# gongweibao/FleetX

Measured on AMD Instinct MI355X. Metric: tokens/sec (whole node) GPT-3 6.7B hybrid-parallel at 1/2/4/8 MI355X, higher is better.
Workload: dtype bf16; 1 GPU; model=gpt3-6.7B, global_batch=8, seq_len=1024, parallelism=dp1, micro_batch=8, hip_graph=True, grad_reduce_dtype=float32, recompute=False

## Files before the change

csrc/kernels/norm_eltwise.hip:

```cpp
#include "fx_api.h"
#include "fx_common.h"

namespace {

struct DropCfg {
  uint32_t klo, khi, thr;
  float scale;
  int enabled;
  const uint64_t* salt;
};

__device__ __forceinline__ DropCfg resolve_drop(DropCfg d) {
  if (d.enabled && d.salt != nullptr) {
    const uint64_t k = salt_key(((uint64_t)d.khi << 32) | d.klo, *d.salt);
    d.klo = (uint32_t)k;
    d.khi = (uint32_t)(k >> 32);
  }
  return d;
}

__device__ __forceinline__ float drop_apply(float v, uint64_t idx, const DropCfg& d) {
  if (!d.enabled) return v;
  uint32_t h = elem_rand_pair(idx, d.klo, d.khi);
  uint32_t r = (idx & 1) ? (h >> 16) : (h & 0xffffu);
  return r >= d.thr ? v * d.scale : 0.f;
}

__device__ __forceinline__ void drop_apply8(float* v, uint64_t idx0, const DropCfg& d) {
  if (!d.enabled) return;
#pragma unroll
  for (int q = 0; q < 4; ++q) {
    const uint32_t h = elem_rand_pair(idx0 + 2 * q, d.klo, d.khi);
    v[2 * q] = (h & 0xffffu) >= d.thr ? v[2 * q] * d.scale : 0.f;
    v[2 * q + 1] = (h >> 16) >= d.thr ? v[2 * q + 1] * d.scale : 0.f;
  }
}

template <typename T, int VPT, bool MASK = false>
__global__ __launch_bounds__(256) void add_ln_fwd_kernel(
    const uint16_t* __restrict__ x, const uint16_t* __restrict__ bias,
    const uint16_t* __restrict__ residual, const uint16_t* __restrict__ gamma,
    const uint16_t* __restrict__ beta, uint16_t* __restrict__ s_out,
    uint16_t* __restrict__ y, float* __restrict__ mean_out, float* __restrict__ rstd_out,
    int rows, int h, float eps, DropCfg drop_) {
  const DropCfg drop = resolve_drop(drop_);
  const int lane = threadIdx.x & 63;
  const int row = blockIdx.x * 4 + (threadIdx.x >> 6);
  if (row >= rows) return;
  const size_t base = (size_t)row * h;
  uint4 xr[VPT], rr[VPT], br[VPT];
#pragma unroll
  for (int i = 0; i < VPT; ++i) {
    const int c = (i * 64 + lane) * 8;
    xr[i] = rr[i] = br[i] = make_uint4(0, 0, 0, 0);
    if (!MASK || c < h) xr[i] = *reinterpret_cast<const uint4*>(x + base + c);
  }
  if (residual) {
#pragma unroll
    for (int i = 0; i < VPT; ++i) {
      const int c = (i * 64 + lane) * 8;
      if (!MASK || c < h) rr[i] = *reinterpret_cast<const uint4*>(residual + base + c);
    }
  }
  if (bias) {
#pragma unroll
    for (int i = 0; i < VPT; ++i) {
      const int c = (i * 64 + lane) * 8;
      if (!MASK || c < h) br[i] = *reinterpret_cast<const uint4*>(bias + c);
    }
  }
  float v[VPT][8];
  float sum = 0.f;
#pragma unroll
  for (int i = 0; i < VPT; ++i) {
    const int c = (i * 64 + lane) * 8;
    if (MASK && c >= h) {
#pragma unroll
      for (int j = 0; j < 8; ++j) v[i][j] = 0.f;
      continue;
    }
    unpack8<T>(xr[i], v[i]);
    if (bias) {
      float b[8];
      unpack8<T>(br[i], b);
#pragma unroll
      for (int j = 0; j < 8; ++j) v[i][j] += b[j];
    }
    if (drop.enabled) {
      drop_apply8(v[i], base + c, drop);
    }
    if (residual) {
      float r[8];
      unpack8<T>(rr[i], r);
#pragma unroll
      for (int j = 0; j < 8; ++j) v[i][j] += r[j];
    }
    if (s_out) {
      store8<T>(s_out + base + c, v[i]);
#pragma unroll
      for (int j = 0; j < 8; ++j) v[i][j] = round_to<T>(v[i][j]);
    }
#pragma unroll
    for (int j = 0; j < 8; ++j) sum += v[i][j];
  }
  const float mean = wave_sum(sum) / h;
  float var = 0.f;
#pragma unroll
  for (int i = 0; i < VPT; ++i) {
    if (MASK && (i * 64 + lane) * 8 >= h) continue;
#pragma unroll
    for (int j = 0; j < 8; ++j) {
      float d = v[i][j] - mean;
      var += d * d;
    }
  }
  const float rstd = rsqrtf(wave_sum(var) / h + eps);
#pragma unroll
  for (int i = 0; i < VPT; ++i) {
    const int c = (i * 64 + lane) * 8;
    if (MASK && c >= h) continue;
    float g[8], b[8], o[8];
    load8<T>(gamma + c, g);
    load8<T>(beta + c, b);
#pragma unroll
    for (int j = 0; j < 8; ++j) o[j] = (v[i][j] - mean) * rstd * g[j] + b[j];
    store8<T>(y + base + c, o);
  }
  if (lane == 0) {
    mean_out[row] = mean;
    rstd_out[row] = rstd;
  }
}

template <typename T>
__global__ __launch_bounds__(256) void add_ln_fwd_generic(
    const uint16_t* __restrict__ x, const uint16_t* __restrict__ bias,
    const uint16_t* __restrict__ residual, const uint16_t* __restrict__ gamma,
    const uint16_t* __restrict__ beta, uint16_t* __restrict__ s_out,
    uint16_t* __restrict__ y, float* __restrict__ mean_out, float* __restrict__ rstd_out,
    int rows, int h, float eps, DropCfg drop_) {
  const DropCfg drop = resolve_drop(drop_);
  const int lane = threadIdx.x & 63;
  const int row = blockIdx.x * 4 + (threadIdx.x >> 6);
  if (row >= rows) return;
  const size_t base = (size_t)row * h;
  const int nv = h / 8;
  auto value = [&](int c, float* v) {
    load8<T>(x + base + c, v);
    if (bias) {
      float b[8];
      load8<T>(bias + c, b);
      for (int j = 0; j < 8; ++j) v[j] += b[j];
    }
    if (drop.enabled)
      drop_apply8(v, base + c, drop);
    if (residual) {
      float r[8];
      load8<T>(residual + base + c, r);
      for (int j = 0; j < 8; ++j) v[j] += r[j];
    }
  };
  float sum = 0.f;
  for (int vi = lane; vi < nv; vi += 64) {
    float v[8];
    value(vi * 8, v);
    if (s_out) {
      store8<T>(s_out + base + vi * 8, v);
      for (int j = 0; j < 8; ++j) v[j] = round_to<T>(v[j]);
    }
    for (int j = 0; j < 8; ++j) sum += v[j];
  }
  const float mean = wave_sum(sum) / h;
  float var = 0.f;
  for (int vi = lane; vi < nv; vi += 64) {
    float v[8];
    if (s_out) load8<T>(s_out + base + vi * 8, v); else value(vi * 8, v);
    for (int j = 0; j < 8; ++j) { float d = v[j] - mean; var += d * d; }
  }
  const float rstd = rsqrtf(wave_sum(var) / h + eps);
  for (int vi = lane; vi < nv; vi += 64) {
    float v[8], g[8], b[8], o[8];
    if (s_out) load8<T>(s_out + base + vi * 8, v); else value(vi * 8, v);
    load8<T>(gamma + vi * 8, g);
    load8<T>(beta + vi * 8, b);
    for (int j = 0; j < 8; ++j) o[j] = (v[j] - mean) * rstd * g[j] + b[j];
    store8<T>(y + base + vi * 8, o);
  }
  if (lane == 0) { mean_out[row] = mean; rstd_out[row] = rstd; }
}

template <typename T, int VPT, bool MASK = false>
__global__ __launch_bounds__(256) void ln_bwd_row_kernel(
    const uint16_t* __restrict__ dy, const uint16_t* __restrict__ s,
    const float* __restrict__ mean_in, const float* __restrict__ rstd_in,
    const uint16_t* __restrict__ gamma, const uint16_t* __restrict__ ds_in,
    uint16_t* __restrict__ ds_out, uint16_t* __restrict__ dx_out, int rows, int h,
    DropCfg drop_) {
  const DropCfg drop = resolve_drop(drop_);
  const int lane = threadIdx.x & 63;
  const int row = blockIdx.x * 4 + (threadIdx.x >> 6);
  if (row >= rows) return;
  const size_t base = (size_t)row * h;
  const float mean = mean_in[row], rstd = rstd_in[row];
  float xh[VPT][8], gdy[VPT][8];
  float s1 = 0.f, s2 = 0.f;
#pragma unroll
  for (int i = 0; i < VPT; ++i) {
    const int c = (i * 64 + lane) * 8;
    if (MASK && c >= h) {
#pragma unroll
      for (int j = 0; j < 8; ++j) xh[i][j] = gdy[i][j] = 0.f;
      continue;
    }
    float a[8], g[8], d[8];
    load8<T>(s + base + c, a);
    load8<T>(gamma + c, g);
    load8<T>(dy + base + c, d);
#pragma unroll
    for (int j = 0; j < 8; ++j) {
      xh[i][j] = (a[j] - mean) * rstd;
      gdy[i][j] = d[j] * g[j];
      s1 += gdy[i][j];
      s2 += gdy[i][j] * xh[i][j];
    }
  }
  uint4 dr[VPT];
  if (ds_in) {
#pragma unroll
    for (int i = 0; i < VPT; ++i) {
      const int c = (i * 64 + lane) * 8;
      dr[i] = make_uint4(0, 0, 0, 0);
      if (!MASK || c < h) dr[i] = *reinterpret_cast<const uint4*>(ds_in + base + c);
    }
  }
  const float m1 = wave_sum(s1) / h, m2 = wave_sum(s2) / h;
#pragma unroll
  for (int i = 0; i < VPT; ++i) {
    const int c = (i * 64 + lane) * 8;
    if (MASK && c >= h) continue;
    float o[8];
#pragma unroll
    for (int j = 0; j < 8; ++j) o[j] = rstd * (gdy[i][j] - m1 - xh[i][j] * m2);
    if (ds_in) {
      float r[8];
      unpack8<T>(dr[i], r);
#pragma unroll
      for (int j = 0; j < 8; ++j) o[j] += r[j];
    }
    store8<T>(ds_out + base + c, o);
    if (drop.enabled) {
      drop_apply8(o, base + c, drop);
      store8<T>(dx_out + base + c, o);
    } else if (dx_out != ds_out) {
      store8<T>(dx_out + base + c, o);
    }
  }
}

template <typename T>
__global__ __launch_bounds__(256) void ln_bwd_row_generic(
    const uint16_t* __restrict__ dy, const uint16_t* __restrict__ s,
    const float* __restrict__ mean_in, const float* __restrict__ rstd_in,
    const uint16_t* __restrict__ gamma, const uint16_t* __restrict__ ds_in,
    uint16_t* __restrict__ ds_out, uint16_t* __restrict__ dx_out, int rows, int h,
    DropCfg drop_) {
  const DropCfg drop = resolve_drop(drop_);
  const int lane = threadIdx.x & 63;
  const int row = blockIdx.x * 4 + (threadIdx.x >> 6);
  if (row >= rows) return;
  const size_t base = (size_t)row * h;
  const float mean = mean_in[row], rstd = rstd_in[row];
  const int nv = h / 8;
  float s1 = 0.f, s2 = 0.f;
  for (int vi = lane; vi < nv; vi += 64) {
    float a[8], g[8], d[8];
    load8<T>(s + base + vi * 8, a);
    load8<T>(gamma + vi * 8, g);
    load8<T>(dy + base + vi * 8, d);
    for (int j = 0; j < 8; ++j) {
      float xh = (a[j] - mean) * rstd, gd = d[j] * g[j];
      s1 += gd;
      s2 += gd * xh;
    }
  }
  const float m1 = wave_sum(s1) / h, m2 = wave_sum(s2) / h;
  for (int vi = lane; vi < nv; vi += 64) {
    const int c = vi * 8;
    float a[8], g[8], d[8], o[8];
    load8<T>(s + base + c, a);
    load8<T>(gamma + c, g);
    load8<T>(dy + base + c, d);
    for (int j = 0; j < 8; ++j) o[j] = rstd * (d[j] * g[j] - m1 - (a[j] - mean) * rstd * m2);
    if (ds_in) {
      float r[8];
      load8<T>(ds_in + base + c, r);
      for (int j = 0; j < 8; ++j) o[j] += r[j];
    }
    store8<T>(ds_out + base + c, o);
    if (drop.enabled) {
      drop_apply8(o, base + c, drop);
      store8<T>(dx_out + base + c, o);
    } else if (dx_out != ds_out) {
      store8<T>(dx_out + base + c, o);
    }
  }
}

template <typename T, int VPT, int WPR, bool MASK, bool DB>
__global__ __launch_bounds__(256, 2) void ln_bwd_cols_kernel(
    const uint16_t* __restrict__ dy, const uint16_t* __restrict__ s,
    const float* __restrict__ mean_in, const float* __restrict__ rstd_in,
    const uint16_t* __restrict__ gamma, const uint16_t* __restrict__ ds_in,
    uint16_t* __restrict__ ds_out, uint16_t* __restrict__ dx_out, int rows, int h,
    int rows_per_group, float* __restrict__ part, DropCfg drop_) {
  constexpr int NG = 4 / WPR;
  __shared__ float red[4 * 512 * VPT];
  __shared__ float xs[2][4][2];
  const DropCfg drop = resolve_drop(drop_);
  const int lane = threadIdx.x & 63, w = threadIdx.x >> 6;
  const int grp = w / WPR, half = w % WPR;
  const int hw = h / WPR, cbase = half * hw;
  const int r0 = min(rows, (blockIdx.x * NG + grp) * rows_per_group);
  const int r1 = min(rows, r0 + rows_per_group);
  uint4 gp[VPT];
  float ag[VPT][8], ab[VPT][8], ax[DB ? VPT : 1][8];
#pragma unroll
  for (int i = 0; i < VPT; ++i) {
    const int c = (i * 64 + lane) * 8;
    gp[i] = (!MASK || c < hw) ? *reinterpret_cast<const uint4*>(gamma + cbase + c)
                              : make_uint4(0, 0, 0, 0);
#pragma unroll
    for (int j = 0; j < 8; ++j) {
      ag[i][j] = ab[i][j] = 0.f;
      if (DB) ax[i][j] = 0.f;
    }
  }
  for (int k = 0; k < rows_per_group; ++k) {
    const int r = r0 + k;
    const bool live = r < r1;
    if (WPR == 1 && !live) break;
    const size_t base = (size_t)(live ? r : 0) * h + cbase;
    uint4 ca[VPT], cd[VPT], cr[VPT];
    float mean = 0.f, rstd = 0.f, s1 = 0.f, s2 = 0.f;
    if (live) {
#pragma unroll
      for (int i = 0; i < VPT; ++i) {
        const int c = (i * 64 + lane) * 8;
        if (MASK && c >= hw) continue;
        ca[i] = *reinterpret_cast<const uint4*>(s + base + c);
        cd[i] = *reinterpret_cast<const uint4*>(dy + base + c);
      }
      if (ds_in) {
#pragma unroll
        for (int i = 0; i < VPT; ++i) {
          const int c = (i * 64 + lane) * 8;
          if (MASK && c >= hw) continue;
          cr[i] = *reinterpret_cast<const uint4*>(ds_in + base + c);
        }
      }
      mean = mean_in[r];
      rstd = rstd_in[r];
#pragma unroll
      for (int i = 0; i < VPT; ++i) {
        const int c = (i * 64 + lane) * 8;
        if (MASK && c >= hw) continue;
        float a[8], d[8], g[8];
        unpack8<T>(ca[i], a);
        unpack8<T>(cd[i], d);
        unpack8<T>(gp[i], g);
#pragma unroll
        for (int j = 0; j < 8; ++j) {
          const float xh = (a[j] - mean) * rstd, gd = d[j] * g[j];
          s1 += gd;
          s2 += gd * xh;
          ag[i][j] += d[j] * xh;
          ab[i][j] += d[j];
        }
      }
    }
    s1 = wave_sum(s1);
    s2 = wave_sum(s2);
    if constexpr (WPR > 1) {
      if (lane == 0) {
        xs[k & 1][w][0] = s1;
        xs[k & 1][w][1] = s2;
      }
      __syncthreads();
      s1 = xs[k & 1][WPR * grp][0];
      s2 = xs[k & 1][WPR * grp][1];
#pragma unroll
      for (int q = 1; q < WPR; ++q) {
        s1 += xs[k & 1][WPR * grp + q][0];
        s2 += xs[k & 1][WPR * grp + q][1];
      }
    }
    if (!live) continue;
    const float m1 = s1 / h, m2 = s2 / h;
#pragma unroll
    for (int i = 0; i < VPT; ++i) {
      const int c = (i * 64 + lane) * 8;
      if (MASK && c >= hw) continue;
      float a[8], d[8], g[8], o[8];
      unpack8<T>(ca[i], a);
      unpack8<T>(cd[i], d);
      unpack8<T>(gp[i], g);
#pragma unroll
      for (int j = 0; j < 8; ++j) o[j] = rstd * (d[j] * g[j] - m1 - (a[j] - mean) * rstd * m2);
      if (ds_in) {
        float rr[8];
        unpack8<T>(cr[i], rr);
#pragma unroll
        for (int j = 0; j < 8; ++j) o[j] += rr[j];
      }
      store8<T>(ds_out + base + c, o);
      if (drop.enabled) {
        drop_apply8(o, base + c, drop);
        store8<T>(dx_out + base + c, o);
      } else if (dx_out != ds_out) {
        store8<T>(dx_out + base + c, o);
      }
      if (DB) {
#pragma unroll
        for (int j = 0; j < 8; ++j) ax[i][j] += round_to<T>(o[j]);
      }
    }
  }
#pragma unroll
  for (int arr = 0; arr < (DB ? 3 : 2); ++arr) {
    __syncthreads();
#pragma unroll
    for (int i = 0; i < VPT; ++i) {
      const int c = (i * 64 + lane) * 8;
      if (MASK && c >= hw) continue;
#pragma unroll
      for (int j = 0; j < 8; ++j)
        red[grp * h + cbase + c + j] = arr == 0 ? ag[i][j] : arr == 1 ? ab[i][j] : ax[DB ? i : 0][j];
    }
    __syncthreads();
    float* out = part + ((size_t)arr * gridDim.x + blockIdx.x) * h;
    for (int c = threadIdx.x; c < h; c += 256) {
      float v = red[c];
#pragma unroll
      for (int q = 1; q < NG; ++q) v += red[q * h + c];
      out[c] = v;
    }
  }
}

struct LnColsOut {
  float* f32[3];
  uint16_t* t16[3];
  int acc[3];
};
template <typename T>
__global__ __launch_bounds__(256) void ln_cols_finalize_kernel(const float* __restrict__ part,
                                                               int G, int h, LnColsOut f) {
  __shared__ float tr[8][132];
  const int arr = blockIdx.y;
  const float* p = part + (size_t)arr * G * h;
  const int q = threadIdx.x & 31, sr = threadIdx.x >> 5;
  const int c0 = blockIdx.x * 128 + q * 4;
  floatx4 acc = {0.f, 0.f, 0.f, 0.f};
  if (c0 < h) {
    for (int k0 = sr; k0 < G; k0 += 128) {
      floatx4 v[16];
#pragma unroll
      for (int u = 0; u < 16; ++u) {
        const int k = k0 + 8 * u;
        v[u] = k < G ? *reinterpret_cast<const floatx4*>(p + (size_t)k * h + c0)
                     : floatx4{0.f, 0.f, 0.f, 0.f};
      }
#pragma unroll
      for (int u = 0; u < 16; ++u) acc += v[u];
    }
  }
#pragma unroll
  for (int j = 0; j < 4; ++j) tr[sr][q * 4 + j] = acc[j];
  __syncthreads();
  const int c = threadIdx.x, gc = blockIdx.x * 128 + c;
  if (c >= 128 || gc >= h) return;
  float sum = 0.f;
#pragma unroll
  for (int t = 0; t < 8; ++t) sum += tr[t][c];
  if (f.f32[arr]) f.f32[arr][gc] = f.acc[arr] ? f.f32[arr][gc] + sum : sum;
  if (f.t16[arr]) f.t16[arr][gc] = Elt<T>::from_f(sum);
}

typedef __attribute__((address_space(1))) float gf32;
typedef __attribute__((address_space(1))) int gi32;

__device__ __forceinline__ void st_part(float* p, float v) {
  __hip_atomic_store((gf32*)p, v, __ATOMIC_RELAXED, __HIP_MEMORY_SCOPE_AGENT);
}

struct ColFin {
  int* cnt;
  float* f32[2];
  uint16_t* t16[2];
  int acc[2];
};

template <typename T>
__device__ __forceinline__ void colsum_tail(const float* __restrict__ p0,
                                            const float* __restrict__ p1, int cols, int np,
                                            const ColFin& f) {
  __shared__ int last;
  asm volatile("s_waitcnt vmcnt(0)" ::: "memory");
  __syncthreads();
  if (threadIdx.x == 0) {
    const int t = __hip_atomic_fetch_add((gi32*)(f.cnt + 32 * blockIdx.x), 1, __ATOMIC_RELAXED,
                                         __HIP_MEMORY_SCOPE_AGENT);
    last = t == (int)gridDim.y - 1;
    if (last)
      __hip_atomic_store((gi32*)(f.cnt + 32 * blockIdx.x), 0, __ATOMIC_RELAXED,
                         __HIP_MEMORY_SCOPE_AGENT);
  }
  __syncthreads();
  if (!last) return;
  __builtin_amdgcn_fence(__ATOMIC_ACQUIRE, "wavefront");
  __shared__ float tr[8][132];
  const int q = threadIdx.x & 31, sr = threadIdx.x >> 5;
  const int c0 = blockIdx.x * 128 + q * 4;
  const int splits = gridDim.y;
  for (int which = 0; which < np; ++which) {
    const float* p = which ? p1 : p0;
    floatx4 s = {0.f, 0.f, 0.f, 0.f};
    if (c0 < cols) {
      const auto rs = __builtin_amdgcn_make_buffer_rsrc(const_cast<float*>(p), 0,
                                                        splits * cols * 4, 0x00020000);
      for (int k0 = sr; k0 < splits; k0 += 128) {
        floatx4 v[16];
#pragma unroll
        for (int u = 0; u < 16; ++u) {
          const int k = k0 + 8 * u;
          const uint32_t off = k < splits ? (uint32_t)(k * cols + c0) * 4u : 0x80000000u;
          v[u] = __builtin_bit_cast(floatx4, __builtin_amdgcn_raw_buffer_load_b128(rs, off, 0, 16));
        }
#pragma unroll
        for (int u = 0; u < 16; ++u) s += v[u];
      }
    }
#pragma unroll
    for (int j = 0; j < 4; ++j) tr[sr][q * 4 + j] = s[j];
    __syncthreads();
    const int c = threadIdx.x, gc = blockIdx.x * 128 + c;
    if (c < 128 && gc < cols) {
      float sum = 0.f;
#pragma unroll
      for (int t = 0; t < 8; ++t) sum += tr[t][c];
      if (f.f32[which]) f.f32[which][gc] = f.acc[which] ? f.f32[which][gc] + sum : sum;
      if (f.t16[which]) f.t16[which][gc] = Elt<T>::from_f(sum);
    }
    __syncthreads();
  }
}

template <typename T, int MODE>
__global__ __launch_bounds__(256) void coltile_partial_kernel(
    const uint16_t* __restrict__ a, const uint16_t* __restrict__ b,
    const float* __restrict__ mean, const float* __restrict__ rstd,
    float* __restrict__ p0, float* __restrict__ p1, int rows, int cols, int rows_per_split,
    ColFin fin) {
  __shared__ float red[2][16][129];
  const int tx = threadIdx.x & 15, ty = threadIdx.x >> 4;
  const int col = blockIdx.x * 128 + tx * 8;
  const int r0 = blockIdx.y * rows_per_split;
  const int r1 = min(rows, r0 + rows_per_split);
  float acc0[8], acc1[8];
#pragma unroll
  for (int j = 0; j < 8; ++j) acc0[j] = acc1[j] = 0.f;
  if (col < cols) {
    int r = r0 + ty;
    for (; r + 48 < r1; r += 64) {
      float va[4][8], vb[MODE == 0 ? 4 : 1][8], m[4], rs[4];
#pragma unroll
      for (int q = 0; q < 4; ++q) {
        const size_t off = (size_t)(r + 16 * q) * cols + col;
        load8<T>(a + off, va[q]);
        if (MODE == 0) {
          load8<T>(b + off, vb[q]);
          m[q] = mean[r + 16 * q];
          rs[q] = rstd[r + 16 * q];
        }
      }
#pragma unroll
      for (int q = 0; q < 4; ++q) {
#pragma unroll
        for (int j = 0; j < 8; ++j) {
          if (MODE == 0) {
            acc0[j] += va[q][j] * (vb[MODE == 0 ? q : 0][j] - m[q]) * rs[q];
            acc1[j] += va[q][j];
          } else {
            acc0[j] += va[q][j];
          }
        }
      }
    }
    for (; r < r1; r += 16) {
      const size_t off = (size_t)r * cols + col;
      float va[8];
      load8<T>(a + off, va);
      if (MODE == 0) {
        float vb[8];
        load8<T>(b + off, vb);
        const float m = mean[r], rs = rstd[r];
#pragma unroll
        for (int j = 0; j < 8; ++j) {
          acc0[j] += va[j] * (vb[j] - m) * rs;
          acc1[j] += va[j];
        }
      } else {
#pragma unroll
        for (int j = 0; j < 8; ++j) acc0[j] += va[j];
      }
    }
  }
#pragma unroll
  for (int j = 0; j < 8; ++j) {
    red[0][ty][tx * 8 + j] = acc0[j];
    red[1][ty][tx * 8 + j] = acc1[j];
  }
  __syncthreads();
  const int which = threadIdx.x >> 7, c = threadIdx.x & 127;
  if (MODE == 0 || which == 0) {
    float s = 0.f;
#pragma unroll
    for (int t = 0; t < 16; ++t) s += red[which][t][c];
    const int gc = blockIdx.x * 128 + c;
    if (gc < cols) st_part((which == 0 ? p0 : p1) + (size_t)blockIdx.y * cols + gc, s);
  }
  if (fin.cnt) colsum_tail<T>(p0, p1, cols, MODE == 0 ? 2 : 1, fin);
}

template <typename T>
__global__ void coltile_finalize_kernel(const float* __restrict__ p, int splits, int cols,
                                        float* __restrict__ out_f32, uint16_t* __restrict__ out_t,
                                        int accumulate) {
  const int c = blockIdx.x * blockDim.x + threadIdx.x;
  if (c >= cols) return;
  float a[8];
#pragma unroll
  for (int j = 0; j < 8; ++j) a[j] = 0.f;
  int k = 0;
  for (; k + 8 <= splits; k += 8) {
#pragma unroll
    for (int j = 0; j < 8; ++j) a[j] += p[(size_t)(k + j) * cols + c];
  }
  for (int j = 0; k + j < splits; ++j) a[j] += p[(size_t)(k + j) * cols + c];
  const float s = ((a[0] + a[1]) + (a[2] + a[3])) + ((a[4] + a[5]) + (a[6] + a[7]));
  if (out_f32) out_f32[c] = accumulate ? out_f32[c] + s : s;
  if (out_t) out_t[c] = Elt<T>::from_f(s);
}

template <typename T, bool ERF>
__global__ __launch_bounds__(256) void bias_gelu_fwd_kernel(
    const uint16_t* __restrict__ x, const uint16_t* __restrict__ bias, uint16_t* __restrict__ y,
    long n8, int cols) {
  for (long v = blockIdx.x * (long)blockDim.x + threadIdx.x; v < n8; v += (long)gridDim.x * blockDim.x) {
    const long off = v * 8;
    const int c = (int)(off % cols);
    float a[8], b[8];
    load8<T>(x + off, a);
    if (bias) load8<T>(bias + c, b);
#pragma unroll
    for (int j = 0; j < 8; ++j) {
      float t = a[j] + (bias ? b[j] : 0.f);
      a[j] = ERF ? gelu_erf(t) : gelu_tanh(t);
    }
    store8<T>(y + off, a);
  }
}

template <typename T, bool ERF>
__global__ __launch_bounds__(256) void bias_gelu_bwd_kernel(
    const uint16_t* __restrict__ dy, const uint16_t* __restrict__ x,
    const uint16_t* __restrict__ bias, uint16_t* __restrict__ dx, float* __restrict__ part,
    int rows, int cols, int rows_per_split, ColFin fin) {
  __shared__ float red[16][129];
  const int tx = threadIdx.x & 15, ty = threadIdx.x >> 4;
  const int col = blockIdx.x * 128 + tx * 8;
  const int r0 = blockIdx.y * rows_per_split;
  const int r1 = min(rows, r0 + rows_per_split);
  float acc[8];
#pragma unroll
  for (int j = 0; j < 8; ++j) acc[j] = 0.f;
  if (col < cols) {
    float b[8];
    if (bias) load8<T>(bias + col, b);
    else {
#pragma unroll
      for (int j = 0; j < 8; ++j) b[j] = 0.f;
    }
    for (int r = r0 + ty; r < r1; r += 16) {
      const size_t off = (size_t)r * cols + col;
      float g[8], a[8];
      load8<T>(dy + off, g);
      load8<T>(x + off, a);
#pragma unroll
      for (int j = 0; j < 8; ++j) {
        float t = a[j] + b[j];
        g[j] *= ERF ? gelu_erf_grad(t) : gelu_tanh_grad(t);
      }
      store8<T>(dx + off, g);
#pragma unroll
      for (int j = 0; j < 8; ++j) acc[j] += round_to<T>(g[j]);
    }
  }
#pragma unroll
  for (int j = 0; j < 8; ++j) red[ty][tx * 8 + j] = acc[j];
  __syncthreads();
  if (threadIdx.x < 128) {
    float s = 0.f;
#pragma unroll
    for (int t = 0; t < 16; ++t) s += red[t][threadIdx.x];
    const int gc = blockIdx.x * 128 + threadIdx.x;
    if (part && gc < cols) st_part(part + (size_t)blockIdx.y * cols + gc, s);
  }
  if (fin.cnt) colsum_tail<T>(part, nullptr, cols, 1, fin);
}

template <typename T>
__global__ __launch_bounds__(256) void bias_dropout_add_fwd_kernel(
    const uint16_t* __restrict__ x, const uint16_t* __restrict__ bias,
    const uint16_t* __restrict__ residual, uint16_t* __restrict__ out, long n8, int cols,
    DropCfg drop_) {
  const DropCfg drop = resolve_drop(drop_);
  for (long v = blockIdx.x * (long)blockDim.x + threadIdx.x; v < n8; v += (long)gridDim.x * blockDim.x) {
    const long off = v * 8;
    const int c = (int)(off % cols);
    float a[8];
    load8<T>(x + off, a);
    if (bias) {
      float b[8];
      load8<T>(bias + c, b);
#pragma unroll
      for (int j = 0; j < 8; ++j) a[j] += b[j];
    }
    drop_apply8(a, (uint64_t)off, drop);
    if (residual) {
      float r[8];
      load8<T>(residual + off, r);
#pragma unroll
      for (int j = 0; j < 8; ++j) a[j] += r[j];
    }
    store8<T>(out + off, a);
  }
}

template <typename T>
__global__ __launch_bounds__(256) void dropout_bwd_colsum_kernel(
    const uint16_t* __restrict__ dout, uint16_t* __restrict__ dx, float* __restrict__ part,
    int rows, int cols, int rows_per_split, DropCfg drop_, ColFin fin) {
  const DropCfg drop = resolve_drop(drop_);
  __shared__ float red[16][129];
  const int tx = threadIdx.x & 15, ty = threadIdx.x >> 4;
  const int col = blockIdx.x * 128 + tx * 8;
  const int r0 = blockIdx.y * rows_per_split;
  const int r1 = min(rows, r0 + rows_per_split);
  float acc[8];
#pragma unroll
  for (int j = 0; j < 8; ++j) acc[j] = 0.f;
  if (col < cols) {
    int r = r0 + ty;
    for (; r + 48 < r1; r += 64) {
      float g[4][8];
#pragma unroll
      for (int q = 0; q < 4; ++q) load8<T>(dout + (size_t)(r + 16 * q) * cols + col, g[q]);
#pragma unroll
      for (int q = 0; q < 4; ++q) {
        const size_t off = (size_t)(r + 16 * q) * cols + col;
        drop_apply8(g[q], off, drop);
        if (dx) {
          store8<T>(dx + off, g[q]);
#pragma unroll
          for (int j = 0; j < 8; ++j) g[q][j] = round_to<T>(g[q][j]);
        }
#pragma unroll
        for (int j = 0; j < 8; ++j) acc[j] += g[q][j];
      }
    }
    for (; r < r1; r += 16) {
      const size_t off = (size_t)r * cols + col;
      float g[8];
      load8<T>(dout + off, g);
      drop_apply8(g, off, drop);
      if (dx) {
        store8<T>(dx + off, g);
#pragma unroll
        for (int j = 0; j < 8; ++j) g[j] = round_to<T>(g[j]);
      }
#pragma unroll
      for (int j = 0; j < 8; ++j) acc[j] += g[j];
    }
  }
#pragma unroll
  for (int j = 0; j < 8; ++j) red[ty][tx * 8 + j] = acc[j];
  __syncthreads();
  if (threadIdx.x < 128) {
    float s = 0.f;
#pragma unroll
    for (int t = 0; t < 16; ++t) s += red[t][threadIdx.x];
    const int gc = blockIdx.x * 128 + threadIdx.x;
    if (part && gc < cols) st_part(part + (size_t)blockIdx.y * cols + gc, s);
  }
  if (fin.cnt) colsum_tail<T>(part, nullptr, cols, 1, fin);
}

template <typename T>
__global__ __launch_bounds__(256) void dropout_fwd_kernel(const uint16_t* __restrict__ x,
                                                          uint16_t* __restrict__ y, long n,
                                                          DropCfg drop_) {
  const DropCfg drop = resolve_drop(drop_);
  const long n8 = n / 8;
  for (long v = blockIdx.x * (long)blockDim.x + threadIdx.x; v < n8; v += (long)gridDim.x * blockDim.x) {
    const long off = v * 8;
    float a[8];
    load8<T>(x + off, a);
    drop_apply8(a, (uint64_t)off, drop);
    store8<T>(y + off, a);
  }
  for (long i = n8 * 8 + blockIdx.x * (long)blockDim.x + threadIdx.x; i < n;
       i += (long)gridDim.x * blockDim.x)
    y[i] = Elt<T>::from_f(drop_apply(Elt<T>::to_f(x[i]), (uint64_t)i, drop));
}

DropCfg make_drop(float p, uint64_t key, const void* salt) {
  DropCfg d;
  d.enabled = p > 0.f ? 1 : 0;
  d.klo = (uint32_t)(key & 0xffffffffu);
  d.khi = (uint32_t)(key >> 32);
  d.thr = (uint32_t)(p * 65536.0f + 0.5f);
  d.scale = p < 1.f ? 1.f / (1.f - p) : 0.f;
  d.salt = reinterpret_cast<const uint64_t*>(salt);
  return d;
}

inline int grid_for(long n8) {
  long g = (n8 + 255) / 256;
  if (g > 8192) g = 8192;
  if (g < 1) g = 1;
  return (int)g;
}

inline int splits_for(int rows, int cols) {
  static const int blocks = [] {
    const char* e = getenv("FLEETX_COLSUM_BLOCKS");
    const int v = e ? atoi(e) : 0;
    return v > 0 ? v : 1024;
  }();
  int tiles = (cols + 127) / 128;
  int s = blocks / (tiles > 0 ? tiles : 1);
  if (s < 1) s = 1;
  int max_s = (rows + 15) / 16;
  if (s > max_s) s = max_s;
  if (s > 512) s = 512;
  return s;
}

}

#define FX_DISPATCH_T(dtype, ...)        \
  if (dtype == 0) {                      \
    using T = bf16;                      \
    __VA_ARGS__;                         \
  } else {                               \
    using T = f16;                       \
    __VA_ARGS__;                         \
  }

static ColFin make_fin(int* cnt, float* f0, void* t0, int acc0, float* f1, void* t1, int acc1) {
  ColFin f;
  f.cnt = cnt;
  f.f32[0] = f0; f.f32[1] = f1;
  f.t16[0] = (uint16_t*)t0; f.t16[1] = (uint16_t*)t1;
  f.acc[0] = acc0; f.acc[1] = acc1;
  return f;
}

extern "C" int fx_coltile_splits(int rows, int cols) { return splits_for(rows, cols); }

extern "C" void fx_add_ln_fwd(int dtype, const void* x, const void* bias, const void* residual,
                              const void* gamma, const void* beta, void* s_out, void* y,
                              float* mean, float* rstd, int rows, int h, float eps, float p,
                              uint64_t key, const void* salt, hipStream_t st) {
  DropCfg d = make_drop(p, key, salt);
  dim3 grid((rows + 3) / 4), block(256);
  auto X = (const uint16_t*)x;
  auto B = (const uint16_t*)bias;
  auto R = (const uint16_t*)residual;
  auto G = (const uint16_t*)gamma;
  auto Be = (const uint16_t*)beta;
  auto S = (uint16_t*)s_out;
  auto Y = (uint16_t*)y;
#define LN_CASE(V)                                                                          \
  case V:                                                                                   \
    FX_DISPATCH_T(dtype, add_ln_fwd_kernel<T, V><<<grid, block, 0, st>>>(                   \
                             X, B, R, G, Be, S, Y, mean, rstd, rows, h, eps, d));           \
    break;
  if (h % 512 == 0 && h / 512 <= 16) {
    switch (h / 512) {
      LN_CASE(1) LN_CASE(2) LN_CASE(3) LN_CASE(4) LN_CASE(5) LN_CASE(6) LN_CASE(7) LN_CASE(8)
      LN_CASE(10) LN_CASE(12) LN_CASE(16)
      default:
        FX_DISPATCH_T(dtype, add_ln_fwd_generic<T><<<grid, block, 0, st>>>(
                                 X, B, R, G, Be, S, Y, mean, rstd, rows, h, eps, d));
    }
  } else if (h % 8 == 0 && h < 8 * 512) {
#define LNM_CASE(V)                                                                          \
  case V:                                                                                    \
    FX_DISPATCH_T(dtype, add_ln_fwd_kernel<T, V, true><<<grid, block, 0, st>>>(              \
                             X, B, R, G, Be, S, Y, mean, rstd, rows, h, eps, d));            \
    break;
    switch ((h + 511) / 512) {
      LNM_CASE(1) LNM_CASE(2) LNM_CASE(3) LNM_CASE(4) LNM_CASE(5) LNM_CASE(6) LNM_CASE(7)
      LNM_CASE(8)
    }
#undef LNM_CASE
  } else {
    FX_DISPATCH_T(dtype, add_ln_fwd_generic<T><<<grid, block, 0, st>>>(
                             X, B, R, G, Be, S, Y, mean, rstd, rows, h, eps, d));
  }
#undef LN_CASE
}

extern "C" void fx_ln_bwd_row(int dtype, const void* dy, const void* s, const float* mean,
                              const float* rstd, const void* gamma, const void* ds_in,
                              void* ds_out, void* dx_out, int rows, int h, float p, uint64_t key,
                              const void* salt, hipStream_t st) {
  DropCfg d = make_drop(p, key, salt);
  dim3 grid((rows + 3) / 4), block(256);
  auto DY = (const uint16_t*)dy;
  auto S = (const uint16_t*)s;
  auto G = (const uint16_t*)gamma;
  auto DI = (const uint16_t*)ds_in;
  auto DS = (uint16_t*)ds_out;
  auto DX = (uint16_t*)dx_out;
#define LNB_CASE(V)                                                                       \
  case V:                                                                                 \
    FX_DISPATCH_T(dtype, ln_bwd_row_kernel<T, V><<<grid, block, 0, st>>>(                 \
                             DY, S, mean, rstd, G, DI, DS, DX, rows, h, d));              \
    break;
  if (h % 512 == 0 && h / 512 <= 8) {
    switch (h / 512) {
      LNB_CASE(1) LNB_CASE(2) LNB_CASE(3) LNB_CASE(4) LNB_CASE(5) LNB_CASE(6) LNB_CASE(7)
      LNB_CASE(8)
      default:
        FX_DISPATCH_T(dtype, ln_bwd_row_generic<T><<<grid, block, 0, st>>>(
                                 DY, S, mean, rstd, G, DI, DS, DX, rows, h, d));
    }
  } else if (h % 8 == 0 && h < 8 * 512) {
#define LNBM_CASE(V)                                                                      \
  case V:                                                                                 \
    FX_DISPATCH_T(dtype, ln_bwd_row_kernel<T, V, true><<<grid, block, 0, st>>>(           \
                             DY, S, mean, rstd, G, DI, DS, DX, rows, h, d));              \
    break;
    switch ((h + 511) / 512) {
      LNBM_CASE(1) LNBM_CASE(2) LNBM_CASE(3) LNBM_CASE(4) LNBM_CASE(5) LNBM_CASE(6)
      LNBM_CASE(7) LNBM_CASE(8)
    }
#undef LNBM_CASE
  } else {
    FX_DISPATCH_T(dtype, ln_bwd_row_generic<T><<<grid, block, 0, st>>>(
                             DY, S, mean, rstd, G, DI, DS, DX, rows, h, d));
  }
#undef LNB_CASE
}

static int ln_cols_wpr(int h) { return h <= 1536 ? 1 : h <= 3072 ? 2 : 4; }
static int ln_cols_rows_per_group(int rows, int h) {
  const int ng = 4 / ln_cols_wpr(h);
  int rpg = (rows + 512 * ng - 1) / (512 * ng);
  return rpg < 2 ? 2 : rpg;
}
extern "C" int fx_ln_bwd_cols_blocks(int rows, int h, int max_h) {
  if (rows <= 0 || h > (max_h < 4096 ? max_h : 4096) || h % (8 * ln_cols_wpr(h))) return 0;
  const int ng = 4 / ln_cols_wpr(h), rpg = ln_cols_rows_per_group(rows, h);
  return (rows + ng * rpg - 1) / (ng * rpg);
}

extern "C" int fx_ln_bwd_cols(int dtype, const void* dy, const void* s, const float* mean,
                              const float* rstd, const void* gamma, const void* ds_in,
                              void* ds_out, void* dx_out, int rows, int h, float p, uint64_t key,
                              float* part, int with_dbias, float* fg, void* tg, int accg,
                              float* fb, void* tb, int accb, float* fx, void* tx, int accx,
                              const void* salt, hipStream_t st) {
  const int G = fx_ln_bwd_cols_blocks(rows, h, 4096);
  if (G == 0) return -1;
  const int wpr = ln_cols_wpr(h), hw = h / wpr;
  const int rpg = ln_cols_rows_per_group(rows, h);
  DropCfg d = make_drop(p, key, salt);
  auto DY = (const uint16_t*)dy;
  auto S = (const uint16_t*)s;
  auto GM = (const uint16_t*)gamma;
  auto DI = (const uint16_t*)ds_in;
  auto DS = (uint16_t*)ds_out;
  auto DX = (uint16_t*)dx_out;
  const int vpt = (hw + 511) / 512;
  const bool mask = hw % 512 != 0;
#define LNC_GO(V, W, M, DB)                                                                   \
  FX_DISPATCH_T(dtype, ln_bwd_cols_kernel<T, V, W, M, DB><<<G, 256, 0, st>>>(                 \
                           DY, S, mean, rstd, GM, DI, DS, DX, rows, h, rpg, part, d))
#define LNC_M(V, W)                                                                           \
  if (mask) {                                                                                 \
    if (with_dbias) { LNC_GO(V, W, true, true); } else { LNC_GO(V, W, true, false); }         \
  } else {                                                                                    \
    if (with_dbias) { LNC_GO(V, W, false, true); } else { LNC_GO(V, W, false, false); }       \
  }
#define LNC_V(V)                                                                              \
  case V:                                                                                     \
    if (wpr == 1) { LNC_M(V, 1) } else if (wpr == 2) { LNC_M(V, 2) } else { LNC_M(V, 4) }     \
    break;
  switch (vpt) {
    LNC_V(1) LNC_V(2) LNC_V(3)
    default: return -1;
  }
#undef LNC_V
#undef LNC_M
#undef LNC_GO
  LnColsOut f;
  f.f32[0] = fg; f.f32[1] = fb; f.f32[2] = fx;
  f.t16[0] = (uint16_t*)tg; f.t16[1] = (uint16_t*)tb; f.t16[2] = (uint16_t*)tx;
  f.acc[0] = accg; f.acc[1] = accb; f.acc[2] = accx;
  dim3 grid((h + 127) / 128, with_dbias ? 3 : 2);
  FX_DISPATCH_T(dtype, ln_cols_finalize_kernel<T><<<grid, 256, 0, st>>>(part, G, h, f));
  return 0;
}

extern "C" void fx_coltile_partial(int dtype, int mode, const void* a, const void* b,
                                   const float* mean, const float* rstd, float* p0, float* p1,
                                   int rows, int cols, int splits, hipStream_t st, int* cnt,
                                   float* f0, void* t0, int acc0, float* f1, void* t1, int acc1) {
  const ColFin fin = make_fin(cnt, f0, t0, acc0, f1, t1, acc1);
  int rps = (rows + splits - 1) / splits;
  dim3 grid((cols + 127) / 128, splits), block(256);
  auto A = (const uint16_t*)a;
  auto B = (const uint16_t*)b;
  if (mode == 0) {
    FX_DISPATCH_T(dtype, coltile_partial_kernel<T, 0><<<grid, block, 0, st>>>(
                             A, B, mean, rstd, p0, p1, rows, cols, rps, fin));
  } else {
    FX_DISPATCH_T(dtype, coltile_partial_kernel<T, 1><<<grid, block, 0, st>>>(
                             A, B, mean, rstd, p0, p1, rows, cols, rps, fin));
  }
}

extern "C" void fx_coltile_finalize(int dtype, const float* part, int splits, int cols,
                                    float* out_f32, void* out_t, int accumulate, hipStream_t st) {
  dim3 grid((cols + 255) / 256), block(256);
  FX_DISPATCH_T(dtype, coltile_finalize_kernel<T><<<grid, block, 0, st>>>(
                           part, splits, cols, out_f32, (uint16_t*)out_t, accumulate));
}

extern "C" void fx_bias_gelu_fwd(int dtype, int erf, const void* x, const void* bias, void* y,
                                 long n, int cols, hipStream_t st) {
  long n8 = n / 8;
  if (erf) {
    FX_DISPATCH_T(dtype, bias_gelu_fwd_kernel<T, true><<<grid_for(n8), 256, 0, st>>>(
                             (const uint16_t*)x, (const uint16_t*)bias, (uint16_t*)y, n8, cols));
  } else {
    FX_DISPATCH_T(dtype, bias_gelu_fwd_kernel<T, false><<<grid_for(n8), 256, 0, st>>>(
                             (const uint16_t*)x, (const uint16_t*)bias, (uint16_t*)y, n8, cols));
  }
}

extern "C" void fx_bias_gelu_bwd(int dtype, int erf, const void* dy, const void* x,
                                 const void* bias, void* dx, float* part, int rows, int cols,
                                 int splits, hipStream_t st, int* cnt, float* out_f32,
                                 void* out_t, int acc) {
  const ColFin fin = make_fin(cnt, out_f32, out_t, acc, nullptr, nullptr, 0);
  int rps = (rows + splits - 1) / splits;
  dim3 grid((cols + 127) / 128, splits), block(256);
  if (erf) {
    FX_DISPATCH_T(dtype, bias_gelu_bwd_kernel<T, true><<<grid, block, 0, st>>>(
                             (const uint16_t*)dy, (const uint16_t*)x, (const uint16_t*)bias,
                             (uint16_t*)dx, part, rows, cols, rps, fin));
  } else {
    FX_DISPATCH_T(dtype, bias_gelu_bwd_kernel<T, false><<<grid, block, 0, st>>>(
                             (const uint16_t*)dy, (const uint16_t*)x, (const uint16_t*)bias,
                             (uint16_t*)dx, part, rows, cols, rps, fin));
  }
}

extern "C" void fx_bias_dropout_add_fwd(int dtype, const void* x, const void* bias,
                                        const void* residual, void* out, long n, int cols, float p,
                                        uint64_t key, const void* salt, hipStream_t st) {
  DropCfg d = make_drop(p, key, salt);
  long n8 = n / 8;
  FX_DISPATCH_T(dtype, bias_dropout_add_fwd_kernel<T><<<grid_for(n8), 256, 0, st>>>(
                           (const uint16_t*)x, (const uint16_t*)bias, (const uint16_t*)residual,
                           (uint16_t*)out, n8, cols, d));
}

extern "C" void fx_dropout_bwd_colsum(int dtype, const void* dout, void* dx, float* part,
                                      int rows, int cols, int splits, float p, uint64_t key,
                                      const void* salt, hipStream_t st, int* cnt,
                                      float* out_f32, void* out_t, int acc) {
  const ColFin fin = make_fin(cnt, out_f32, out_t, acc, nullptr, nullptr, 0);
  DropCfg d = make_drop(p, key, salt);
  int rps = (rows + splits - 1) / splits;
  dim3 grid((cols + 127) / 128, splits), block(256);
  FX_DISPATCH_T(dtype, dropout_bwd_colsum_kernel<T><<<grid, block, 0, st>>>(
                           (const uint16_t*)dout, (uint16_t*)dx, part, rows, cols, rps, d, fin));
}

extern "C" void fx_dropout_fwd(int dtype, const void* x, void* y, long n, float p, uint64_t key,
                               const void* salt, hipStream_t st) {
  DropCfg d = make_drop(p, key, salt);
  long n8 = n / 8;
  FX_DISPATCH_T(dtype, dropout_fwd_kernel<T><<<grid_for(n8), 256, 0, st>>>(
                           (const uint16_t*)x, (uint16_t*)y, n, d));
}
```

fleetx_amd/ops/norm.py:

```python
import os

import torch

from . import _lib
from ..parallel import grad_sink as sink, rng as _rng


_TICKETS = {}


def colsum_tickets(device, cols):
    st = torch.cuda.current_stream(device).cuda_stream
    need = 32 * ((cols + 127) // 128)
    t = _TICKETS.get(st)
    if t is None or t.numel() < need:
        t = torch.zeros(max(4096, need), dtype=torch.int32, device=device)
        _TICKETS[st] = t
    return t.data_ptr()


_TARGET_KW = (("f0", "t0", "acc0"), ("f1", "t1", "acc1"))


def _coltile(mode, x, aux, rows, cols, targets):
    k = _lib.kernels()
    splits = k.coltile_splits(rows, cols)
    p0 = torch.empty(splits, cols, device=x.device, dtype=torch.float32)
    p1 = torch.empty_like(p0) if mode == 0 else None
    fin = {}
    for (kf, kt, ka), (f32, t16, acc) in zip(_TARGET_KW, targets):
        if f32:
            fin[kf], fin[ka] = f32, acc
        else:
            fin[kt] = t16
    k.coltile_partial(_lib.dt_code(x.dtype), mode, x.data_ptr(), *aux, p0.data_ptr(),
                      _lib.ptr(p1), rows, cols, splits, _lib.stream(),
                      cnt=colsum_tickets(x.device, cols), **fin)


def _col_target(prm, direct, cols, like):
    if direct:
        mg, acc = sink.open_write(prm)
        return (mg.data_ptr(), 0, int(acc)), None
    g = torch.empty(cols, device=like.device, dtype=like.dtype)
    return (0, g.data_ptr(), 0), g


def col_sum(x, cols):
    if not _lib.vec8_ok(cols, x):
        return x.reshape(-1, cols).float().sum(0).to(x.dtype)
    out = torch.empty(cols, device=x.device, dtype=x.dtype)
    _coltile(1, x, (0, 0, 0), x.numel() // cols, cols, [(0, out.data_ptr(), 0)])
    return out


def col_sum_f32(x, dst, accumulate=False):
    cols = dst.numel()
    x = x.contiguous()
    if not _lib.vec8_ok(cols, x):
        sink.store_or_add(dst, x.reshape(-1, cols).float().sum(0).view_as(dst), accumulate)
        return dst
    if dst.dtype != torch.float32 or not dst.is_contiguous():
        raise ValueError("col_sum_f32: dst must be contiguous fp32")
    _coltile(1, x, (0, 0, 0), x.numel() // cols, cols, [(dst.data_ptr(), 0, int(accumulate))])
    return dst


def _dropout_ref(x, p, key):
    if p <= 0.0:
        return x
    m = _rng.keep_mask(x.shape, p, key, x.device)
    return torch.where(m, x * (1.0 / (1.0 - p)), torch.zeros_like(x))


def _ln_bwd_cols_max_h():
    mode = os.environ.get("FLEETX_LN_BWD_FUSED", "1")
    return {"0": 0, "2": 4096}.get(mode, 1536)


def _ln_bwd_cols(k, dc, dy, s, mean, rstd, weight, ctx, ds_in, ds, dx, rows, h):
    G = k.ln_bwd_cols_blocks(rows, h, 4096)
    with_db = bool(ctx.has_bias)
    part = torch.empty(3 if with_db else 2, G, h, device=dy.device, dtype=torch.float32)
    prms = (weight, ctx.lnbias, ctx.bias if with_db else None)
    outs, grads = [], []
    for prm in prms:
        t, g = ((0, 0, 0), None) if prm is None else \
            _col_target(prm, sink.fused(prm, fp32_contiguous=True), h, dy)
        outs.append(t)
        grads.append(g)
    (fg, tg, ag), (fb, tb, ab), (fx, tx, ax) = outs
    rc = k.ln_bwd_cols(dc, dy.data_ptr(), s.data_ptr(), mean.data_ptr(), rstd.data_ptr(),
                       weight.data_ptr(), _lib.ptr(ds_in), ds.data_ptr(), dx.data_ptr(), rows, h,
                       float(ctx.p), ctx.key, part.data_ptr(), int(with_db), fg, tg, ag, fb, tb,
                       ab, fx, tx, ax, _rng.device_salt_ptr(), _lib.stream())
    if rc != 0:
        raise RuntimeError("ln_bwd_cols: shape rows=%d h=%d not covered" % (rows, h))
    for prm, (f32, _, _) in zip(prms, outs):
        if f32:
            sink.close_write(prm)
    return grads


class _AddLayerNorm(torch.autograd.Function):
    @staticmethod
    def forward(ctx, x, bias, residual, weight, lnbias, eps, p, key, store_sum):
        h = x.shape[-1]
        rows = x.numel() // h
        ctx.p, ctx.key, ctx.has_bias, ctx.has_res = p, key, bias is not None, residual is not None
        ctx.h = h
        x = x.contiguous()
        if _lib.vec8_ok(h, x, bias, residual, weight, lnbias):
            k = _lib.kernels()
            fused = bias is not None or residual is not None or p > 0
            s = torch.empty_like(x) if fused else None
            y = torch.empty_like(x)
            mean = torch.empty(rows, device=x.device, dtype=torch.float32)
            rstd = torch.empty_like(mean)
            k.add_ln_fwd(_lib.dt_code(x.dtype), x.data_ptr(), _lib.ptr(bias), _lib.ptr(residual),
                         weight.data_ptr(), lnbias.data_ptr(), _lib.ptr(s), y.data_ptr(),
                         mean.data_ptr(), rstd.data_ptr(), rows, h, float(eps), float(p), key,
                         _rng.device_salt_ptr(), _lib.stream())
            s_saved = s if s is not None else x
            if s is None and store_sum:
                s = x
        else:
            v = x
            if bias is not None or residual is not None or p > 0:
                v = x.float() if bias is None else x.float() + bias.float()
                v = _dropout_ref(v, p, key)
                if residual is not None:
                    v = v + residual.float()
                v = v.to(x.dtype)
            s_saved = v
            s = v if (store_sum or bias is not None or residual is not None or p > 0) else None
            vf = v.float()
            mean = vf.mean(-1).reshape(-1)
            var = ((vf - mean.view(*vf.shape[:-1], 1)) ** 2).mean(-1).reshape(-1)
            rstd = torch.rsqrt(var + eps)
            y = ((vf - mean.view(*vf.shape[:-1], 1)) * rstd.view(*vf.shape[:-1], 1) * weight.float()
                 + lnbias.float()).to(x.dtype)
        ctx.save_for_backward(s_saved, mean, rstd, weight)
        ctx.lnbias, ctx.bias = lnbias, bias
        ctx.return_sum = s is not None
        if s is None:
            return y
        return s, y

    @staticmethod
    def backward(ctx, *grads):
        if ctx.return_sum:
            ds_in, dy = grads
        else:
            ds_in, dy = None, grads[0]
        s, mean, rstd, weight = ctx.saved_tensors
        h = ctx.h
        rows = s.numel() // h
        dy = dy.contiguous()
        if ds_in is not None:
            ds_in = ds_in.contiguous()
        if _lib.vec8_ok(h, dy, ds_in, s, weight):
            k = _lib.kernels()
            dc = _lib.dt_code(dy.dtype)
            ds = torch.empty_like(dy)
            dx = torch.empty_like(dy) if ctx.p > 0 else ds
            if k.ln_bwd_cols_blocks(rows, h, _ln_bwd_cols_max_h()) > 0:
                dw, db, dbias = _ln_bwd_cols(k, dc, dy, s, mean, rstd, weight, ctx, ds_in, ds, dx,
                                             rows, h)
                dres = ds if ctx.has_res else None
                return dx, dbias, dres, dw, db, None, None, None, None
            k.ln_bwd_row(dc, dy.data_ptr(), s.data_ptr(), mean.data_ptr(), rstd.data_ptr(),
                         weight.data_ptr(), _lib.ptr(ds_in), ds.data_ptr(), dx.data_ptr(), rows, h,
                         float(ctx.p), ctx.key, _rng.device_salt_ptr(), _lib.stream())
            direct = sink.fused(weight) and sink.fused(ctx.lnbias)
            (tw, dw), (tb, db) = (_col_target(prm, direct, h, dy) for prm in (weight, ctx.lnbias))
            _coltile(0, dy, (s.data_ptr(), mean.data_ptr(), rstd.data_ptr()), rows, h, [tw, tb])
            if direct:
                sink.close_write(weight)
                sink.close_write(ctx.lnbias)
            dbias = None
            if ctx.has_bias:
                if sink.fused(ctx.bias):
                    mg, acc = sink.open_write(ctx.bias)
                    col_sum_f32(dx, mg, acc)
                    sink.close_write(ctx.bias)
                else:
                    dbias = col_sum(dx, h)
        else:
            sf = s.float().reshape(rows, h)
            xh = (sf - mean.view(rows, 1)) * rstd.view(rows, 1)
            g = dy.float().reshape(rows, h) * weight.float()
            m1 = g.mean(-1, keepdim=True)
            m2 = (g * xh).mean(-1, keepdim=True)
            dsf = rstd.view(rows, 1) * (g - m1 - xh * m2)
            if ds_in is not None:
                dsf = dsf + ds_in.float().reshape(rows, h)
            ds = dsf.to(dy.dtype).reshape(dy.shape)
            dx = _dropout_ref(ds, ctx.p, ctx.key)
            dw = sink.deliver(weight, (dy.float().reshape(rows, h) * xh).sum(0), weight.dtype,
                              on_gpu=True)
            db = sink.deliver(ctx.lnbias, dy.float().reshape(rows, h).sum(0), weight.dtype,
                              on_gpu=True)
            dbias = None
            if ctx.has_bias:
                dbias = sink.deliver(ctx.bias, dx.float().reshape(rows, h).sum(0), dy.dtype,
                                     on_gpu=True)
        dres = ds if ctx.has_res else None
        return dx, dbias, dres, dw, db, None, None, None, None


def add_layer_norm(x, bias, residual, weight, lnbias, eps=1e-5, p=0.0, key=0):
    return _AddLayerNorm.apply(x, bias, residual, weight, lnbias, eps, p, key, True)


def layer_norm(x, weight, bias, eps=1e-5):
    return _AddLayerNorm.apply(x, None, None, weight, bias, eps, 0.0, 0, False)


def layer_norm_keep_input(x, weight, bias, eps=1e-5):
    return _AddLayerNorm.apply(x, None, None, weight, bias, eps, 0.0, 0, True)


class FusedLayerNorm(torch.nn.Module):

    def __init__(self, hidden, eps=1e-5, dtype=None, device=None):
        super().__init__()
        self.weight = torch.nn.Parameter(torch.ones(hidden, dtype=dtype, device=device))
        self.bias = torch.nn.Parameter(torch.zeros(hidden, dtype=dtype, device=device))
        self.weight._fx_fused_wgrad_ok = True
        self.bias._fx_fused_wgrad_ok = True
        self.eps = eps
        self.normalized_shape = (hidden,)

    def forward(self, x):
        return layer_norm(x, self.weight, self.bias, self.eps)
```

Baseline: 28040 tokens/s.

## Software-pipeline row loads in fused LN backward and enable it for hidden 4096

Restructures the fused LayerNorm-backward column kernel so multi-wave-per-row variants can prefetch upcoming rows into a small register ring before processing the current one. The single-wave path is split out without the dead-row bookkeeping. The Python dispatch now routes hidden size 4096 (GPT-3 6.7B) to the fused row+column kernel by default instead of the separate row kernel plus column-sum tiles. The ring raises register pressure, and the new default path for width 4096 may reduce occupancy compared with the old two-kernel route.

Result: no change. 28150 tokens/s (median of 6 runs) (+0.4%).

```diff
diff --git a/csrc/kernels/norm_eltwise.hip b/csrc/kernels/norm_eltwise.hip
--- a/csrc/kernels/norm_eltwise.hip
+++ b/csrc/kernels/norm_eltwise.hip
@@ -306,6 +306,9 @@
   }
 }
 
+#ifndef LN_COLS_DEPTH
+#define LN_COLS_DEPTH 1
+#endif
 template <typename T, int VPT, int WPR, bool MASK, bool DB>
 __global__ __launch_bounds__(256, 2) void ln_bwd_cols_kernel(
     const uint16_t* __restrict__ dy, const uint16_t* __restrict__ s,
@@ -314,6 +317,7 @@
     uint16_t* __restrict__ ds_out, uint16_t* __restrict__ dx_out, int rows, int h,
     int rows_per_group, float* __restrict__ part, DropCfg drop_) {
   constexpr int NG = 4 / WPR;
+  constexpr int D = VPT == 3 && !MASK ? 0 : LN_COLS_DEPTH;
   __shared__ float red[4 * 512 * VPT];
   __shared__ float xs[2][4][2];
   const DropCfg drop = resolve_drop(drop_);
@@ -335,14 +339,13 @@
       if (DB) ax[i][j] = 0.f;
     }
   }
-  for (int k = 0; k < rows_per_group; ++k) {
-    const int r = r0 + k;
-    const bool live = r < r1;
-    if (WPR == 1 && !live) break;
-    const size_t base = (size_t)(live ? r : 0) * h + cbase;
-    uint4 ca[VPT], cd[VPT], cr[VPT];
-    float mean = 0.f, rstd = 0.f, s1 = 0.f, s2 = 0.f;
-    if (live) {
+  if constexpr (WPR == 1) {
+    for (int k = 0; k < rows_per_group; ++k) {
+      const int r = r0 + k;
+      if (r >= r1) break;
+      const size_t base = (size_t)r * h + cbase;
+      uint4 ca[VPT], cd[VPT], cr[VPT];
+      float s1 = 0.f, s2 = 0.f;
 #pragma unroll
       for (int i = 0; i < VPT; ++i) {
         const int c = (i * 64 + lane) * 8;
@@ -358,8 +361,7 @@
           cr[i] = *reinterpret_cast<const uint4*>(ds_in + base + c);
         }
       }
-      mean = mean_in[r];
-      rstd = rstd_in[r];
+      const float mean = mean_in[r], rstd = rstd_in[r];
 #pragma unroll
       for (int i = 0; i < VPT; ++i) {
         const int c = (i * 64 + lane) * 8;
@@ -377,10 +379,93 @@
           ab[i][j] += d[j];
         }
       }
-    }
-    s1 = wave_sum(s1);
-    s2 = wave_sum(s2);
-    if constexpr (WPR > 1) {
+      s1 = wave_sum(s1);
+      s2 = wave_sum(s2);
+      const float m1 = s1 / h, m2 = s2 / h;
+#pragma unroll
+      for (int i = 0; i < VPT; ++i) {
+        const int c = (i * 64 + lane) * 8;
+        if (MASK && c >= hw) continue;
+        float a[8], d[8], g[8], o[8];
+        unpack8<T>(ca[i], a);
+        unpack8<T>(cd[i], d);
+        unpack8<T>(gp[i], g);
+#pragma unroll
+        for (int j = 0; j < 8; ++j) o[j] = rstd * (d[j] * g[j] - m1 - (a[j] - mean) * rstd * m2);
+        if (ds_in) {
+          float rr[8];
+          unpack8<T>(cr[i], rr);
+#pragma unroll
+          for (int j = 0; j < 8; ++j) o[j] += rr[j];
+        }
+        store8<T>(ds_out + base + c, o);
+        if (drop.enabled) {
+          drop_apply8(o, base + c, drop);
+          store8<T>(dx_out + base + c, o);
+        } else if (dx_out != ds_out) {
+          store8<T>(dx_out + base + c, o);
+        }
+        if (DB) {
+#pragma unroll
+          for (int j = 0; j < 8; ++j) ax[i][j] += round_to<T>(o[j]);
+        }
+      }
+    }
+  } else {
+    struct Row {
+      uint4 a[VPT], d[VPT], r[VPT];
+      float mean, rstd;
+    };
+    auto issue = [&](Row& x, const int k) __attribute__((always_inline)) {
+      if (D == 0 && r0 + k >= r1) return;
+      const int r = min(r0 + k, rows - 1);
+      const size_t base = (size_t)r * h + cbase;
+#pragma unroll
+      for (int i = 0; i < VPT; ++i) {
+        const int c = (i * 64 + lane) * 8;
+        if (MASK && c >= hw) continue;
+        x.a[i] = *reinterpret_cast<const uint4*>(s + base + c);
+        x.d[i] = *reinterpret_cast<const uint4*>(dy + base + c);
+      }
+      if (ds_in) {
+#pragma unroll
+        for (int i = 0; i < VPT; ++i) {
+          const int c = (i * 64 + lane) * 8;
+          if (MASK && c >= hw) continue;
+          x.r[i] = *reinterpret_cast<const uint4*>(ds_in + base + c);
+        }
+      }
+      x.mean = mean_in[r];
+      x.rstd = rstd_in[r];
+    };
+    auto work = [&](const Row& x, const int k) __attribute__((always_inline)) {
+      const int r = r0 + k;
+      const bool live = r < r1;
+      const size_t base = (size_t)(live ? r : 0) * h + cbase;
+      float mean = 0.f, rstd = 0.f, s1 = 0.f, s2 = 0.f;
+      if (live) {
+        mean = x.mean;
+        rstd = x.rstd;
+#pragma unroll
+        for (int i = 0; i < VPT; ++i) {
+          const int c = (i * 64 + lane) * 8;
+          if (MASK && c >= hw) continue;
+          float a[8], d[8], g[8];
+          unpack8<T>(x.a[i], a);
+          unpack8<T>(x.d[i], d);
+          unpack8<T>(gp[i], g);
+#pragma unroll
+          for (int j = 0; j < 8; ++j) {
+            const float xh = (a[j] - mean) * rstd, gd = d[j] * g[j];
+            s1 += gd;
+            s2 += gd * xh;
+            ag[i][j] += d[j] * xh;
+            ab[i][j] += d[j];
+          }
+        }
+      }
+      s1 = wave_sum(s1);
+      s2 = wave_sum(s2);
       if (lane == 0) {
         xs[k & 1][w][0] = s1;
         xs[k & 1][w][1] = s2;
@@ -393,35 +478,54 @@
         s1 += xs[k & 1][WPR * grp + q][0];
         s2 += xs[k & 1][WPR * grp + q][1];
       }
-    }
-    if (!live) continue;
-    const float m1 = s1 / h, m2 = s2 / h;
-#pragma unroll
-    for (int i = 0; i < VPT; ++i) {
-      const int c = (i * 64 + lane) * 8;
-      if (MASK && c >= hw) continue;
-      float a[8], d[8], g[8], o[8];
-      unpack8<T>(ca[i], a);
-      unpack8<T>(cd[i], d);
-      unpack8<T>(gp[i], g);
-#pragma unroll
-      for (int j = 0; j < 8; ++j) o[j] = rstd * (d[j] * g[j] - m1 - (a[j] - mean) * rstd * m2);
-      if (ds_in) {
-        float rr[8];
-        unpack8<T>(cr[i], rr);
-#pragma unroll
-        for (int j = 0; j < 8; ++j) o[j] += rr[j];
-      }
-      store8<T>(ds_out + base + c, o);
-      if (drop.enabled) {
-        drop_apply8(o, base + c, drop);
-        store8<T>(dx_out + base + c, o);
-      } else if (dx_out != ds_out) {
-        store8<T>(dx_out + base + c, o);
-      }
-      if (DB) {
-#pragma unroll
-        for (int j = 0; j < 8; ++j) ax[i][j] += round_to<T>(o[j]);
+      if (!live) return;
+      const float m1 = s1 / h, m2 = s2 / h;
+#pragma unroll
+      for (int i = 0; i < VPT; ++i) {
+        const int c = (i * 64 + lane) * 8;
+        if (MASK && c >= hw) continue;
+        float a[8], d[8], g[8], o[8];
+        unpack8<T>(x.a[i], a);
+        unpack8<T>(x.d[i], d);
+        unpack8<T>(gp[i], g);
+#pragma unroll
+        for (int j = 0; j < 8; ++j) o[j] = rstd * (d[j] * g[j] - m1 - (a[j] - mean) * rstd * m2);
+        if (ds_in) {
+          float rr[8];
+          unpack8<T>(x.r[i], rr);
+#pragma unroll
+          for (int j = 0; j < 8; ++j) o[j] += rr[j];
+        }
+        store8<T>(ds_out + base + c, o);
+        if (drop.enabled) {
+          drop_apply8(o, base + c, drop);
+          store8<T>(dx_out + base + c, o);
+        } else if (dx_out != ds_out) {
+          store8<T>(dx_out + base + c, o);
+        }
+        if (DB) {
+#pragma unroll
+          for (int j = 0; j < 8; ++j) ax[i][j] += round_to<T>(o[j]);
+        }
+      }
+    };
+    if constexpr (D == 0) {
+      for (int k = 0; k < rows_per_group; ++k) {
+        Row x;
+        issue(x, k);
+        work(x, k);
+      }
+    } else {
+      Row ring[D + 1];
+#pragma unroll
+      for (int j = 0; j < D; ++j) issue(ring[j], j);
+      for (int k0 = 0; k0 < rows_per_group; k0 += D + 1) {
+#pragma unroll
+        for (int j = 0; j <= D; ++j) {
+          if (k0 + j >= rows_per_group) break;
+          issue(ring[(j + D) % (D + 1)], k0 + j + D);
+          work(ring[j], k0 + j);
+        }
       }
     }
   }
diff --git a/fleetx_amd/ops/norm.py b/fleetx_amd/ops/norm.py
--- a/fleetx_amd/ops/norm.py
+++ b/fleetx_amd/ops/norm.py
@@ -73,9 +73,12 @@
     return torch.where(m, x * (1.0 / (1.0 - p)), torch.zeros_like(x))
 
 
-def _ln_bwd_cols_max_h():
+_LN_BWD_COLS_WIDE = (4096,)
+
+
+def _ln_bwd_cols_max_h(h):
     mode = os.environ.get("FLEETX_LN_BWD_FUSED", "1")
-    return {"0": 0, "2": 4096}.get(mode, 1536)
+    return {"0": 0, "2": 4096}.get(mode, 4096 if h in _LN_BWD_COLS_WIDE else 1536)
 
 
 def _ln_bwd_cols(k, dc, dy, s, mean, rstd, weight, ctx, ds_in, ds, dx, rows, h):
@@ -164,7 +167,7 @@
             dc = _lib.dt_code(dy.dtype)
             ds = torch.empty_like(dy)
             dx = torch.empty_like(dy) if ctx.p > 0 else ds
-            if k.ln_bwd_cols_blocks(rows, h, _ln_bwd_cols_max_h()) > 0:
+            if k.ln_bwd_cols_blocks(rows, h, _ln_bwd_cols_max_h(h)) > 0:
                 dw, db, dbias = _ln_bwd_cols(k, dc, dy, s, mean, rstd, weight, ctx, ds_in, ds, dx,
                                              rows, h)
                 dres = ds if ctx.has_res else None
```
